# chalkydri/chalkydri

Hardware: AMD Instinct MI355X
Metric: frames/sec (detect+pose) on 1280x800 batch; HBM GB/s vs roofline (higher is better)
Workload: dtype u8 (threshold/segment/clusters: integer; quad fit/decode/SQPnP: f64)

## Files before the change

chalkydri_amd/csrc/k_clusters.hip:

```cpp
#include "ck_internal.h"
#include "ck_emit_row.h"

namespace {

constexpr int NT = 256;
constexpr int ETW = 64, ETH = 16;
constexpr int LW = ETW + 2, LH = ETH + 1;
constexpr int LHT = 512;
constexpr uint32_t SKIP = 0xFFFFFFFFu;

__device__ __forceinline__ uint32_t key_hash(unsigned long long k) {
    uint32_t x = (uint32_t)((k >> 32) ^ k);
    x *= 2654435761u;
    return x ^ (x >> 15);
}

struct EmitArgs {
    const uint8_t *thresh;
    const ck_label_t *labels;
    const uint32_t *groot, *gsize;
    size_t slots;
    int w, h, tiles_x, tiles_y, min_comp;
    int ccl_tiles_x;
    int stop_after;
    int twins;
    ck_stage_ws ws;
};

__device__ __forceinline__ void lds_barrier() { asm volatile("s_waitcnt lgkmcnt(0)\n\ts_barrier" ::: "memory"); }

__global__ __launch_bounds__(NT) void k_emit(EmitArgs a) {
    __shared__ uint8_t sT[LH][LW + 2];
    __shared__ uint32_t sR[LH][LW];
    __shared__ unsigned long long sKey[LHT];
    __shared__ uint32_t sCnt[LHT], sSlot[LHT], sTBase[LHT];
    __shared__ uint32_t sWave[NT / 64 + 1], sRunW[NT / 64 + 1];
    const int tid = threadIdx.x;
    const int tiles = a.tiles_x * a.tiles_y;
    const int frame = blockIdx.x / tiles, tile = blockIdx.x - frame * tiles;
    const int ty = tile / a.tiles_x, tx = tile - ty * a.tiles_x;
    const int x0 = tx * ETW, y0 = ty * ETH;
    const int w = a.w, h = a.h;
    const size_t npix = (size_t)w * h;
    const uint8_t *T = a.thresh + (size_t)frame * npix;
    const ck_label_t *L = a.labels + (size_t)frame * npix;
    const uint32_t *GR = a.groot + (size_t)frame * a.slots, *GS = a.gsize + (size_t)frame * a.slots;
    const ck_stage_ws &ws = a.ws;
    unsigned long long *gkeys = ws.d_ht_keys + (size_t)frame * ws.ht_size;
    unsigned long long *gcount = ws.d_ht_count + (size_t)frame * ws.ht_size;
    uint32_t *counters = ws.d_counters + (size_t)frame * CK_CNT_STRIDE;
    ck_packed_point *tmp = ws.d_tmp + (size_t)frame * ws.ext_cap;
    ck_run *runs = ws.d_runs + (size_t)frame * ws.run_cap;

    for (int i = tid; i < LHT; i += NT) { sKey[i] = 0ull; sCnt[i] = 0; }
    {
        constexpr int SPT = (LH * LW + NT - 1) / NT;
        uint32_t lab[SPT], hop[SPT], csz[SPT], slot[SPT];
        uint8_t tv[SPT];
#pragma unroll
        for (int q = 0; q < SPT; q++) {
            const int i = tid + q * NT;
            const int ly = i / LW, lx = i - ly * LW;
            const int gy = y0 + ly, gx = x0 - 1 + lx;
            tv[q] = 127; lab[q] = CK_LBL_NONE; slot[q] = 0;
            if (i < LH * LW && gy < h && gx >= 0 && gx < w) {
                const uint32_t p = (uint32_t)gy * (uint32_t)w + (uint32_t)gx;
                tv[q] = T[p]; lab[q] = L[p];
                slot[q] = ck_label_slot(lab[q], gx, gy, a.ccl_tiles_x);
            }
        }
#pragma unroll
        for (int q = 0; q < SPT; q++) {
            const bool two = tv[q] != 127 && !(lab[q] & CK_LBL_SMALL) && (lab[q] & CK_LBL_BORDER);
            hop[q] = two ? GR[slot[q]] : CK_LBL_INVALID;
            csz[q] = two ? GS[slot[q]] : 0u;
        }
#pragma unroll
        for (int q = 0; q < SPT; q++) {
            const int i = tid + q * NT;
            if (i >= LH * LW) continue;
            const int ly = i / LW, lx = i - ly * LW;
            uint32_t r = SKIP;
            if (tv[q] != 127 && !(lab[q] & CK_LBL_SMALL)) {
                if (lab[q] & CK_LBL_BORDER) r = ((int)csz[q] < a.min_comp) ? SKIP : hop[q];
                else r = ck_label_interior_root(lab[q], x0 - 1 + lx, y0 + ly, w);
            }
            sT[ly][lx] = tv[q];
            sR[ly][lx] = r;
        }
    }
    lds_barrier();
    if (a.stop_after == 0) return;

    const int lx = (tid & 63) + 1;
    const int gx = x0 + (tid & 63);
    const int row0 = (tid >> 6) * 4;
    const int dxs[4] = {1, 0, -1, 1}, dys[4] = {0, 1, 1, 1};
    const bool colok = gx >= 1 && gx <= w - 2;

    constexpr uint32_t NONE = 0xFFFFFFFFu;
    uint32_t cand[16];
#pragma unroll
    for (int q = 0; q < 16; q++) cand[q] = NONE;
    if (colok) {
#pragma unroll
        for (int rr = 0; rr < 4; rr++) {
            int ly = row0 + rr, gy = y0 + ly;
            if (gy < 1 || gy > h - 2) continue;
            int v0 = sT[ly][lx];
            uint32_t r0 = sR[ly][lx];
            if (r0 == SKIP) continue;
            uint32_t r1v[4];
            bool ok[4];
#pragma unroll
            for (int k = 0; k < 4; k++) {
                const int v1 = sT[ly + dys[k]][lx + dxs[k]];
                r1v[k] = sR[ly + dys[k]][lx + dxs[k]];
                ok[k] = (v0 + v1 == 255) && r1v[k] != SKIP;
            }
#pragma unroll
            for (int k = 0; k < 4; k++) {
                bool leader = ok[k];
#pragma unroll
                for (int j = 0; j < k; j++) leader = leader && !(ok[j] && r1v[j] == r1v[k]);
                if (!leader) continue;
                uint32_t n = 1;
#pragma unroll
                for (int j = k + 1; j < 4; j++) n += (ok[j] && r1v[j] == r1v[k]) ? 1u : 0u;
                const uint32_t r1 = r1v[k];
                unsigned long long key = r0 < r1 ? ((unsigned long long)r0 << 32) | r1 : ((unsigned long long)r1 << 32) | r0;
                uint32_t s = key_hash(key) & (LHT - 1);
                bool placed = false;
                for (int probe = 0; probe < LHT; probe++) {
                    __asm__ volatile("" ::: "memory");
                    unsigned long long prev = sKey[s];
                    if (prev == 0ull) prev = atomicCAS(&sKey[s], 0ull, key);
                    if (prev == 0ull || prev == key) {
                        uint32_t c = (s << 16) | atomicAdd(&sCnt[s], n);
                        cand[rr * 4 + k] = c;
#pragma unroll
                        for (int j = k + 1; j < 4; j++)
                            if (ok[j] && r1v[j] == r1) cand[rr * 4 + j] = ++c;
                        placed = true;
                        break;
                    }
                    s = (s + 1) & (LHT - 1);
                }
                if (!placed) atomicOr(&counters[CK_CNT_STATUS], (uint32_t)CK_FRAME_CLUSTERS_OVERFLOW);
            }
        }
    }
    lds_barrier();
    if (a.stop_after == 1) return;

    const unsigned long long k0 = sKey[2 * tid], k1 = sKey[2 * tid + 1];
    const uint32_t c0 = k0 ? sCnt[2 * tid] : 0u, c1 = k1 ? sCnt[2 * tid + 1] : 0u;
    uint32_t found0 = SKIP, found1 = SKIP, ridx0;
    {
        const uint32_t incl = wave_scan_u32(c0 + c1);
        const unsigned long long b0 = __ballot(k0 != 0ull), b1 = __ballot(k1 != 0ull);
        const unsigned long long below = (1ull << (tid & 63)) - 1ull;
        ridx0 = (uint32_t)(__popcll(b0 & below) + __popcll(b1 & below));
        if ((tid & 63) == 63) sWave[tid >> 6] = incl;
        if ((tid & 63) == 0) sRunW[tid >> 6] = (uint32_t)(__popcll(b0) + __popcll(b1));
        lds_barrier();
        uint32_t before = 0, total = 0, rbefore = 0, rtotal = 0;
#pragma unroll
        for (int wv = 0; wv < NT / 64; wv++) {
            uint32_t t = sWave[wv], r = sRunW[wv];
            if (wv < (tid >> 6)) { before += t; rbefore += r; }
            total += t; rtotal += r;
        }
        ridx0 += rbefore;
        lds_barrier();
        if (tid == 0) {
            sWave[NT / 64] = total ? atomicAdd(&counters[CK_CNT_TMP], total) : 0u;
            sRunW[NT / 64] = rtotal ? atomicAdd(&counters[CK_CNT_RUNS], rtotal) : 0u;
        }
        const uint32_t excl = before + incl - (c0 + c1);
        sTBase[2 * tid] = excl; sTBase[2 * tid + 1] = excl + c0;
        {
            const uint32_t hm = (uint32_t)(ws.ht_size - 1);
            const uint32_t g0 = key_hash(k0) & hm, g1 = key_hash(k1) & hm;
            const unsigned long long p0 = k0 ? atomicCAS(&gkeys[g0], 0ull, k0) : 0ull;
            const unsigned long long p1 = k1 ? atomicCAS(&gkeys[g1], 0ull, k1) : 0ull;
#pragma unroll
            for (int q = 0; q < 2; q++) {
                const unsigned long long key = q ? k1 : k0, pv = q ? p1 : p0;
                if (key == 0ull) continue;
                uint32_t g = q ? g1 : g0, found = SKIP;
                if (pv == 0ull || pv == key) found = g;
                else {
                    for (int probe = 1; probe < ws.ht_size; probe++) {
                        g = (g + 1) & hm;
                        unsigned long long prev = atomicCAS(&gkeys[g], 0ull, key);
                        if (prev == 0ull || prev == key) { found = g; break; }
                    }
                }
                if (found == SKIP) atomicOr(&counters[CK_CNT_STATUS], (uint32_t)CK_FRAME_CLUSTERS_OVERFLOW);
                sSlot[2 * tid + q] = found;
                if (q) found1 = found; else found0 = found;
            }
        }
        if (found0 != SKIP) atomicAdd(&gcount[found0], ((unsigned long long)c0 << 32) | c0);
        if (found1 != SKIP) atomicAdd(&gcount[found1], ((unsigned long long)c1 << 32) | c1);
    }
    lds_barrier();
    if (a.stop_after == 2) return;

    const uint32_t tile_base = sWave[NT / 64];
    if (colok) {
#pragma unroll
        for (int rr = 0; rr < 4; rr++) {
            int ly = row0 + rr, gy = y0 + ly;
#pragma unroll
            for (int k = 0; k < 4; k++) {
                const uint32_t cd = cand[rr * 4 + k];
                if (cd == NONE) continue;
                const uint32_t s = cd >> 16, lr = cd & 0xFFFFu;
                uint32_t slot = sSlot[s];
                if (slot == SKIP) continue;
                uint32_t ti = tile_base + sTBase[s] + lr;
                if (ti >= (uint32_t)ws.point_cap) { atomicOr(&counters[CK_CNT_STATUS], (uint32_t)CK_FRAME_POINTS_OVERFLOW); continue; }
                int v0 = sT[ly][lx], v1 = sT[ly + dys[k]][lx + dxs[k]];
                tmp[ti] = ((uint32_t)(2 * gx + dxs[k]) << 16) | ((uint32_t)(2 * gy + dys[k]) << 3) | ((uint32_t)k << 1) | (v1 > v0 ? 1u : 0u);
            }
        }
    }
    {
        uint32_t ri = sRunW[NT / 64] + ridx0;
#pragma unroll
        for (int q = 0; q < 2; q++) {
            if ((q ? k1 : k0) == 0ull) continue;
            const uint32_t found = q ? found1 : found0;
            if (ri < (uint32_t)ws.run_cap) {
                ck_run r;
                r.slot = found != SKIP ? found : 0u; r.base = 0; r.tmp_start = tile_base + sTBase[2 * tid + q];
                r.count = found != SKIP ? (q ? c1 : c0) : 0u;
                runs[ri] = r;
            } else if (found != SKIP) atomicOr(&counters[CK_CNT_STATUS], (uint32_t)CK_FRAME_CLUSTERS_OVERFLOW);
            ri++;
        }
    }
}

constexpr uint32_t ID_WHITE = 0x40000000u, ID_VALUE = 0x3FFFFFFFu;
static_assert(ID_WHITE == CK_PT_TWIN_SIGN, "a twin's sign is its white neighbour's colour bit, taken as it stands");
constexpr int SR_PAD = ((LH * LW + NT - 1) / NT) * NT;
static_assert(SKIP == CK_ER_SKIP && ID_WHITE == CK_ER_WHITE, "ck_emit_row.h speaks of the staged words of this kernel");
__device__ const ck_emit_row_table g_emit_rows = ck_make_emit_row_table();
static_assert(CK_ER_ROWS == 4 * NT, "one uint4 of the row table per thread");

__global__ __launch_bounds__(NT) __attribute__((amdgpu_num_sgpr(80), amdgpu_waves_per_eu(8))) void k_emit2(EmitArgs a, int xcd_map, int n_frames) {
    __shared__ __attribute__((aligned(16))) uint32_t sRaw[SR_PAD + LHT * 2 + LHT];
    __shared__ uint32_t sSlot[LHT], sTBase[LHT];
    __shared__ uint32_t sWave[NT / 64 + 1], sRunW[NT / 64 + 1];
    __shared__ __attribute__((aligned(16))) uint32_t sRow[CK_ER_ROWS];
    uint32_t *sR = sRaw;
    unsigned long long *sKey = reinterpret_cast<unsigned long long *>(sRaw + SR_PAD);
    uint32_t *sCnt = sRaw + SR_PAD + LHT * 2;
    const int tid = threadIdx.x;
    const int tiles = a.tiles_x * a.tiles_y;
    int frame, tile;
    if (xcd_map) {
        const int x = blockIdx.x & 7, j = blockIdx.x >> 3;
        frame = (j / tiles) * 8 + x; tile = j % tiles;
        if (frame >= n_frames) return;
    } else { frame = blockIdx.x / tiles; tile = blockIdx.x - frame * tiles; }
    const int ty = tile / a.tiles_x, tx = tile - ty * a.tiles_x;
    const int x0 = tx * ETW, y0 = ty * ETH;
    const int w = a.w, h = a.h;
    const size_t npix = (size_t)w * h;
    const uint8_t *T = a.thresh + (size_t)frame * npix;
    const ck_label_t *L = a.labels + (size_t)frame * npix;
    const uint32_t *GR = a.groot + (size_t)frame * a.slots, *GS = a.gsize + (size_t)frame * a.slots;
    const ck_stage_ws &ws = a.ws;
    unsigned long long *gkeys = ws.d_ht_keys + (size_t)frame * ws.ht_size;
    unsigned long long *gcount = ws.d_ht_count + (size_t)frame * ws.ht_size;
    uint32_t *counters = ws.d_counters + (size_t)frame * CK_CNT_STRIDE;
    ck_packed_point *tmp = ws.d_tmp + (size_t)frame * ws.ext_cap;
    ck_run *runs = ws.d_runs + (size_t)frame * ws.run_cap;

    for (int i = tid; i < LHT; i += NT) { sKey[i] = 0ull; sCnt[i] = 0; }
    {
        constexpr int SPT = SR_PAD / NT;
        uint32_t lab[SPT], tv[SPT], slot[SPT], hop[SPT], csz[SPT];
        bool inb[SPT];
        int gxs[SPT], gys[SPT];
#pragma unroll
        for (int q = 0; q < SPT; q++) {
            const int i = tid + q * NT;
            const int ly = i / LW, lx = i - ly * LW;
            const int gy = y0 + ly, gx = x0 - 1 + lx;
            inb[q] = i < LH * LW && gy < h && gx >= 0 && gx < w;
            const int cy = min(gy, h - 1), cx = min(max(gx, 0), w - 1);
            const uint32_t p = (uint32_t)cy * (uint32_t)w + (uint32_t)cx;
            tv[q] = T[p]; lab[q] = L[p];
            gxs[q] = cx; gys[q] = cy;
        }
#pragma unroll
        for (int q = 0; q < SPT; q++) {
            const bool two = inb[q] && tv[q] != 127u && !(lab[q] & CK_LBL_SMALL) && (lab[q] & CK_LBL_BORDER);
            slot[q] = two ? ck_label_slot(lab[q], gxs[q], gys[q], a.ccl_tiles_x) : 0u;
            hop[q] = GR[slot[q]]; csz[q] = GS[slot[q]];
        }
#pragma unroll
        for (int q = 0; q < SPT; q++) {
            const bool brd = (lab[q] & CK_LBL_BORDER) != 0u;
            const bool none = !inb[q] || tv[q] == 127u || (lab[q] & CK_LBL_SMALL) || (brd && (int)csz[q] < a.min_comp);
            const uint32_t root = brd ? hop[q] : ck_label_interior_root(lab[q], gxs[q], gys[q], w);
            sR[tid + q * NT] = none ? SKIP : (root | (tv[q] == 255u ? ID_WHITE : 0u));
        }
    }
    reinterpret_cast<uint4 *>(sRow)[tid] = reinterpret_cast<const uint4 *>(g_emit_rows.e)[tid];
    lds_barrier();
    if (a.stop_after == 0) return;

    const int lx = (tid & 63) + 1;
    const int gx = x0 + (tid & 63);
    const int row0 = (tid >> 6) * 4;

    constexpr uint32_t NONE = 0xFFFFFFFFu;
    uint32_t cand[16];
    {
        uint32_t R[5][3];
        unsigned long long last_key = 0ull;
        uint32_t last_s = 0;
        auto stage_row = [&](int r) {
#pragma unroll
            for (int c = 0; c < 3; c++) R[r][c] = sR[(row0 + r) * LW + lx - 1 + c];
        };
        stage_row(0); stage_row(1);
        uint32_t H[5];
        H[0] = ck_er_hword(R[0][0], R[0][1], R[0][2]);
        const uint32_t colskip = (uint32_t)(((gx - 1) | (w - 2 - gx)) >> 31);
        const uint32_t can = (a.twins ? 3u : 0u) & ~(((uint32_t)((gx - 2) >> 31) & CK_ER_CAN_DROP) | ((uint32_t)((w - 3 - gx) >> 31) & CK_ER_CAN_ABSORB));
        auto count = [&](uint32_t r0, uint32_t r1, uint32_t mult) -> uint32_t {
            const uint32_t ra = r0 & ID_VALUE, rb = r1 & ID_VALUE;
            const unsigned long long key = ra < rb ? ((unsigned long long)ra << 32) | rb : ((unsigned long long)rb << 32) | ra;
            uint32_t s = key_hash(key) & (LHT - 1);
            bool placed = false;
            if (key == last_key) { placed = true; s = last_s; }
            else
            for (int probe = 0; probe < LHT; probe++) {
                __asm__ volatile("" ::: "memory");
                unsigned long long prev = sKey[s];
                if (prev == 0ull) prev = atomicCAS(&sKey[s], 0ull, key);
                if (prev == 0ull || prev == key) { placed = true; break; }
                s = (s + 1) & (LHT - 1);
            }
            if (!placed) { atomicOr(&counters[CK_CNT_STATUS], (uint32_t)CK_FRAME_CLUSTERS_OVERFLOW); return NONE; }
            last_key = key; last_s = s;
            return (s << 16) | (atomicAdd(&sCnt[s], mult) >> 16);
        };
#pragma unroll
        for (int rr = 0; rr < 4; rr++) {
            const int gy = y0 + row0 + rr;
            if (rr < 3) stage_row(rr + 2);
            H[rr + 1] = ck_er_hword(R[rr + 1][0], R[rr + 1][1], R[rr + 1][2]);
            const uint32_t r0 = R[rr][1] | colskip | (uint32_t)(((gy - 1) | (h - 2 - gy)) >> 31);
            const uint32_t r1v[4] = {R[rr][2], R[rr + 1][1], R[rr + 1][0], R[rr + 1][2]};
            uint32_t absorb;
            const uint32_t idx = ck_er_index(H[rr], H[rr + 1], r0, R[rr][0], R[rr][1], R[rr][2], R[rr + 1][0], R[rr + 1][1], R[rr + 1][2], can, &absorb);
            const uint32_t e = sRow[idx];
            const uint32_t lj[4] = {0u, (e >> 20) & 1u, (e >> 21) & 3u, (e >> 23) & 3u};
            uint32_t c4[4] = {NONE, NONE, NONE, NONE};
            uint32_t le = e & CK_ER_LEADERS;
            for (uint32_t j = 0; (le & 0x1Cu) != 0u; j++, le >>= 5) {
                const uint32_t sl = le & 3u;
                const uint32_t r1 = sl == 0u ? r1v[0] : (sl == 1u ? r1v[1] : (sl == 2u ? r1v[2] : r1v[3]));
                const uint32_t c = count(r0, r1, ((le >> 2) & 7u) * 0x10001u + (lj[3] == j ? absorb : 0u));
#pragma unroll
                for (int k = 0; k < 4; k++) c4[k] = lj[k] == j ? c : c4[k];
            }
#pragma unroll
            for (int k = 0; k < 4; k++) {
                const uint32_t nth = k == 0 ? 0u : (k == 1 ? (e >> 25) & 1u : (k == 2 ? (e >> 26) & 3u : (e >> 28) & 3u));
                uint32_t c = c4[k];
                c = ((idx >> (9 - k)) & 1u) ? c : NONE;
                const uint32_t sign = (r1v[k] & ID_WHITE) << 1;
                const uint32_t twin = k == 3 ? (0u - absorb) & (CK_PT_TWIN | (r1v[1] & ID_WHITE)) : 0u;
                cand[rr * 4 + k] = c != NONE ? ((c + nth) | sign | twin) : NONE;
                asm volatile("" : "+v"(cand[rr * 4 + k]));
            }
        }
    }
    lds_barrier();
    if (a.stop_after == 1) return;

    const unsigned long long k0 = sKey[2 * tid], k1 = sKey[2 * tid + 1];
    const uint32_t b0 = k0 ? sCnt[2 * tid] : 0u, b1 = k1 ? sCnt[2 * tid + 1] : 0u;
    const uint32_t c0 = b0 >> 16, c1 = b1 >> 16;
    uint32_t found0 = SKIP, found1 = SKIP, ridx0;
    {
        const uint32_t incl2 = wave_scan_u32(b0 + b1), incl = incl2 >> 16;
        const unsigned long long u0 = __ballot(k0 != 0ull), u1 = __ballot(k1 != 0ull);
        const unsigned long long below = (1ull << (tid & 63)) - 1ull;
        ridx0 = (uint32_t)(__popcll(u0 & below) + __popcll(u1 & below));
        if ((tid & 63) == 63) sWave[tid >> 6] = incl2;
        if ((tid & 63) == 0) sRunW[tid >> 6] = (uint32_t)(__popcll(u0) + __popcll(u1));
        lds_barrier();
        uint32_t before = 0, total = 0, rbefore = 0, rtotal = 0;
#pragma unroll
        for (int wv = 0; wv < NT / 64; wv++) {
            uint32_t t = sWave[wv], r = sRunW[wv];
            if (wv < (tid >> 6)) { before += t; rbefore += r; }
            total += t; rtotal += r;
        }
        ridx0 += rbefore;
        before >>= 16;
        if (tid == 0) {
            const uint32_t ptotal = total >> 16, ltotal = total & 0xFFFFu;
            static_assert(CK_CNT_TMP == 0 && CK_CNT_CLUSTERS == 1 && CK_CNT_STRIDE % 2 == 0, "the two counters are one aligned 64-bit word");
            const unsigned long long was = total ? atomicAdd(reinterpret_cast<unsigned long long *>(counters), ((unsigned long long)ltotal << 32) | ptotal) : 0ull;
            sWave[NT / 64] = (uint32_t)was;
            sRunW[NT / 64] = rtotal ? atomicAdd(&counters[CK_CNT_RUNS], rtotal) : 0u;
            if ((uint32_t)(was >> 32) + ltotal > (uint32_t)ws.point_cap) atomicOr(&counters[CK_CNT_STATUS], (uint32_t)CK_FRAME_POINTS_OVERFLOW);
        }
        const uint32_t excl = before + incl - (c0 + c1);
        sTBase[2 * tid] = excl; sTBase[2 * tid + 1] = excl + c0;
        {
            const uint32_t hm = (uint32_t)(ws.ht_size - 1);
            const uint32_t g0 = key_hash(k0) & hm, g1 = key_hash(k1) & hm;
            const unsigned long long p0 = k0 ? atomicCAS(&gkeys[g0], 0ull, k0) : 0ull;
            const unsigned long long p1 = k1 ? atomicCAS(&gkeys[g1], 0ull, k1) : 0ull;
#pragma unroll
            for (int q = 0; q < 2; q++) {
                const unsigned long long key = q ? k1 : k0, pv = q ? p1 : p0;
                uint32_t found = SKIP;
                if (key != 0ull) {
                    uint32_t g = q ? g1 : g0;
                    if (pv == 0ull || pv == key) found = g;
                    else {
                        for (int probe = 1; probe < ws.ht_size; probe++) {
                            g = (g + 1) & hm;
                            unsigned long long prev = atomicCAS(&gkeys[g], 0ull, key);
                            if (prev == 0ull || prev == key) { found = g; break; }
                        }
                    }
                    if (found == SKIP) atomicOr(&counters[CK_CNT_STATUS], (uint32_t)CK_FRAME_CLUSTERS_OVERFLOW);
                }
                sSlot[2 * tid + q] = found;
                if (q) found1 = found; else found0 = found;
            }
        }
        if (found0 != SKIP) atomicAdd(&gcount[found0], ((unsigned long long)(b0 & 0xFFFFu) << 32) | c0);
        if (found1 != SKIP) atomicAdd(&gcount[found1], ((unsigned long long)(b1 & 0xFFFFu) << 32) | c1);
    }
    lds_barrier();
    if (a.stop_after == 2) return;

    const uint32_t tile_base = sWave[NT / 64];
#pragma unroll
    for (int q = 0; q < 16; q++) {
        const uint32_t cd = cand[q];
        if (cd == NONE) continue;
        const int rr = q >> 2, k = q & 3;
        const int dxk = k == 1 ? 0 : (k == 2 ? -1 : 1), dyk = k == 0 ? 0 : 1;
        const uint32_t s = (cd >> 16) & 0x3FFu, lr = cd & 0xFFFFu;
        if (sSlot[s] == SKIP) continue;
        const uint32_t ti = tile_base + sTBase[s] + lr;
        if (ti >= (uint32_t)ws.point_cap) continue;
        const int gy = y0 + row0 + rr;
        const uint32_t twin = k == 3 ? cd & (CK_PT_TWIN | CK_PT_TWIN_SIGN) : 0u;
        tmp[ti] = twin | ((uint32_t)(2 * gx + dxk) << 16) | ((uint32_t)(2 * gy + dyk) << 3) | ((uint32_t)k << 1) | (cd >> 31);
    }
    {
        uint32_t ri = sRunW[NT / 64] + ridx0;
#pragma unroll
        for (int q = 0; q < 2; q++) {
            if ((q ? k1 : k0) == 0ull) continue;
            const uint32_t found = q ? found1 : found0;
            if (ri < (uint32_t)ws.run_cap) {
                ck_run r;
                r.slot = found != SKIP ? found : 0u; r.base = 0; r.tmp_start = tile_base + (q ? sTBase[2 * tid + 1] : sTBase[2 * tid]);
                r.count = found != SKIP ? (q ? c1 : c0) : 0u;
                runs[ri] = r;
            } else if (found != SKIP) atomicOr(&counters[CK_CNT_STATUS], (uint32_t)CK_FRAME_CLUSTERS_OVERFLOW);
            ri++;
        }
    }
}

__global__ __launch_bounds__(NT) void k_clear(uint4 *keys4, size_t nkeys4, uint4 *cnt4, size_t ncnt4, uint32_t *c0, uint32_t n0, uint32_t *c1,
                                              uint32_t n1, uint32_t *c2, uint32_t n2) {
    const size_t i = (size_t)blockIdx.x * NT + threadIdx.x;
    const uint4 z = make_uint4(0, 0, 0, 0);
    if (i < nkeys4) keys4[i] = z;
    else if (i - nkeys4 < ncnt4) cnt4[i - nkeys4] = z;
    if (i < n0) c0[i] = 0;
    if (i < n1) c1[i] = 0;
    if (i < n2) c2[i] = 0;
}

constexpr int SNT = 1024;
__global__ __launch_bounds__(SNT) void k_scan(ck_stage_ws ws, int min_cluster, int max_cluster) {
    __shared__ uint32_t sPts[SNT / 64], sLog[SNT / 64], sCl[SNT / 64];
    const int frame = blockIdx.x, tid = threadIdx.x, lane = tid & 63, wv = tid >> 6;
    const unsigned long long *gkeys = ws.d_ht_keys + (size_t)frame * ws.ht_size;
    const unsigned long long *gcount = ws.d_ht_count + (size_t)frame * ws.ht_size;
    uint32_t *goff = ws.d_ht_off + (size_t)frame * ws.ht_size;
    uint32_t *counters = ws.d_counters + (size_t)frame * CK_CNT_STRIDE;
    ck_cluster_t *clusters = ws.d_clusters + (size_t)frame * ws.cluster_cap;
    const int seg = ws.ht_size / (SNT / 64);
    const int base = wv * seg;
    uint32_t pts = 0, lpts = 0, cl = 0;
#pragma unroll 8
    for (int r = 0; r < seg; r += 64) {
        const unsigned long long c2 = gcount[base + r + lane];
        const uint32_t c = (uint32_t)c2, lc = (uint32_t)(c2 >> 32);
        bool ok = (int)lc >= min_cluster && (int)lc <= max_cluster;
        pts += ok ? c : 0u; lpts += ok ? lc : 0u; cl += ok ? 1u : 0u;
    }
    pts = (uint32_t)__builtin_amdgcn_readlane((int)wave_scan_u32(pts), 63);
    lpts = (uint32_t)__builtin_amdgcn_readlane((int)wave_scan_u32(lpts), 63);
    cl = (uint32_t)__builtin_amdgcn_readlane((int)wave_scan_u32(cl), 63);
    if (lane == 0) { sPts[wv] = pts; sLog[wv] = lpts; sCl[wv] = cl; }
    __syncthreads();
    uint32_t po = 0, lo = 0, co = 0;
    for (int k = 0; k < wv; k++) { po += sPts[k]; lo += sLog[k]; co += sCl[k]; }
    for (int r4 = 0; r4 < seg; r4 += 256) {
        unsigned long long c4[4];
#pragma unroll
        for (int q = 0; q < 4; q++) c4[q] = r4 + 64 * q < seg ? gcount[base + r4 + 64 * q + lane] : 0ull;
#pragma unroll
    for (int q = 0; q < 4; q++) {
        const int r = r4 + 64 * q;
        if (r >= seg) continue;
        const int e = base + r + lane;
        const uint32_t c = (uint32_t)c4[q], lc = (uint32_t)(c4[q] >> 32);
        const bool ok = (int)lc >= min_cluster && (int)lc <= max_cluster;
        const uint32_t ip = wave_scan_u32(ok ? c : 0u), il = wave_scan_u32(ok ? lc : 0u), ic = wave_scan_u32(ok ? 1u : 0u);
        uint32_t off = SKIP;
        if (ok) {
            const uint32_t my_po = po + ip - c, my_lo = lo + il - lc, my_co = co + ic - 1u;
            if (my_co < (uint32_t)ws.cluster_cap && my_lo + lc <= (uint32_t)ws.point_cap) {
                off = my_po;
                unsigned long long key = gkeys[e];
                ck_cluster_t ck;
                ck.rep0 = (uint32_t)(key >> 32); ck.rep1 = (uint32_t)key; ck.start = my_po; ck.count = c;
                clusters[my_co] = ck;
            } else {
                if (my_co < (uint32_t)ws.cluster_cap) {
                    ck_cluster_t ck;
                    ck.rep0 = 0; ck.rep1 = 0; ck.start = 0; ck.count = 0;
                    clusters[my_co] = ck;
                }
                atomicOr(&counters[CK_CNT_STATUS], (uint32_t)CK_FRAME_CLUSTERS_OVERFLOW);
            }
        }
        goff[e] = off;
        po += (uint32_t)__builtin_amdgcn_readlane((int)ip, 63);
        lo += (uint32_t)__builtin_amdgcn_readlane((int)il, 63);
        co += (uint32_t)__builtin_amdgcn_readlane((int)ic, 63);
    }
    }
    if (tid == SNT - 1) {
        counters[CK_CNT_CLUSTERS] = min(co, (uint32_t)ws.cluster_cap);
        counters[CK_CNT_POINTS] = min(po, (uint32_t)ws.point_cap);
    }
}

template <int RPW>
__global__ __launch_bounds__(NT) void k_scatter(ck_stage_ws ws) {
    const int frame = blockIdx.y;
    const uint32_t *counters = ws.d_counters + (size_t)frame * CK_CNT_STRIDE;
    const uint32_t nruns = min(counters[CK_CNT_RUNS], (uint32_t)ws.run_cap);
    const uint32_t ntmp = min(counters[CK_CNT_TMP], (uint32_t)ws.point_cap);
    const ck_packed_point *tmp = ws.d_tmp + (size_t)frame * ws.ext_cap;
    const ck_run *runs = ws.d_runs + (size_t)frame * ws.run_cap;
    uint32_t *goff = ws.d_ht_off + (size_t)frame * ws.ht_size;
    ck_packed_point *pts = ws.d_points + (size_t)frame * ws.ext_cap;
    const int lane = threadIdx.x & 63;
    const uint32_t wave = blockIdx.x * (NT / 64) + (threadIdx.x >> 6), nwaves = gridDim.x * (NT / 64);
    for (uint32_t r0 = wave * RPW; r0 < nruns; r0 += nwaves * RPW) {
        ck_run mine = {0, 0, 0, 0};
        uint32_t moff = SKIP;
        if (lane < RPW && r0 + lane < nruns) { mine = runs[r0 + lane]; moff = goff[mine.slot]; }
        if (moff == SKIP) mine.count = 0;
        const uint32_t dst0 = mine.count ? atomicAdd(&goff[mine.slot], mine.count) : 0u;
        const unsigned long long small = __ballot(mine.count > 0 && mine.count <= 64);
        unsigned long long todo = small;
        const int sub = lane >> 4, sl = lane & 15;
        while (todo) {
            unsigned long long t = todo;
            int pick = -1;
#pragma unroll
            for (int q = 0; q < 4; q++) {
                const int bit = t ? __builtin_ctzll(t) : -1;
                if (q == sub) pick = bit;
                if (t) t &= t - 1;
            }
            todo = t;
            const int srcl = pick < 0 ? 0 : pick;
            const uint32_t cnt = (uint32_t)__shfl((int)mine.count, srcl, 64), ts = (uint32_t)__shfl((int)mine.tmp_start, srcl, 64),
                           ds = (uint32_t)__shfl((int)dst0, srcl, 64);
            ck_packed_point v[4];
            bool ok[4];
#pragma unroll
            for (int q = 0; q < 4; q++) {
                const uint32_t j = (uint32_t)sl + 16u * q;
                ok[q] = pick >= 0 && j < cnt && ts + j < ntmp;
                v[q] = ok[q] ? tmp[ts + j] : 0u;
            }
#pragma unroll
            for (int q = 0; q < 4; q++)
                if (ok[q]) pts[ds + (uint32_t)sl + 16u * q] = v[q];
        }
        unsigned long long big = __ballot(mine.count > 64);
        while (big) {
            const int srcl = __builtin_ctzll(big);
            big &= big - 1;
            const uint32_t cnt = (uint32_t)__builtin_amdgcn_readlane((int)mine.count, srcl), ts = (uint32_t)__builtin_amdgcn_readlane((int)mine.tmp_start, srcl),
                           ds = (uint32_t)__builtin_amdgcn_readlane((int)dst0, srcl);
            for (uint32_t j0 = 0; j0 < cnt; j0 += 256) {
                ck_packed_point v[4];
                bool ok[4];
#pragma unroll
                for (int q = 0; q < 4; q++) {
                    const uint32_t j = j0 + (uint32_t)lane + 64u * q;
                    ok[q] = j < cnt && ts + j < ntmp;
                    v[q] = ok[q] ? tmp[ts + j] : 0u;
                }
#pragma unroll
                for (int q = 0; q < 4; q++)
                    if (ok[q]) pts[ds + j0 + (uint32_t)lane + 64u * q] = v[q];
            }
        }
    }
}

}

int ck_launch_clusters(ck_handle *h, int n) {
    ck_stage_ws &ws = h->ws;
    {
        const ck_fit_layout fl = ck_fit_scratch_layout(ws, h->cfg.max_batch);
        const size_t nkeys4 = (size_t)ws.ht_size * n / 2, ncnt4 = (size_t)ws.ht_size * n / 2;
        const size_t total4 = nkeys4 + ncnt4;
        hipLaunchKernelGGL(k_clear, dim3((unsigned)((total4 + NT - 1) / NT)), dim3(NT), 0, h->stream,
                           reinterpret_cast<uint4 *>(ws.d_ht_keys), nkeys4, reinterpret_cast<uint4 *>(ws.d_ht_count), ncnt4, ws.d_counters,
                           (uint32_t)(CK_CNT_STRIDE * n), fl.list_counts, 32u, fl.cand_count, (uint32_t)n);
    }
    EmitArgs a;
    a.thresh = h->d_thresh; a.labels = h->d_labels; a.groot = h->d_groot; a.gsize = h->d_gsize; a.slots = (size_t)h->broot_cap;
    a.w = h->qw; a.h = h->qh; a.tiles_x = (h->qw + ETW - 1) / ETW; a.tiles_y = (h->qh + ETH - 1) / ETH;
    a.min_comp = h->cfg.min_component_px; a.ws = ws; a.ccl_tiles_x = h->tiles_x;
    { static const int stop_after = CK_KNOB("CK_EMIT_STOP_AFTER", 99); a.stop_after = stop_after; }
    { static const int twins = CK_KNOB("CK_EMIT_TWINS", 1); a.twins = twins; }
    static const int emit_v = CK_KNOB("CK_EMIT_V", 2);
    static const int emit_xcd = CK_KNOB("CK_EMIT_XCD", -1);
    if (emit_v == 1) hipLaunchKernelGGL(k_emit, dim3((unsigned)(a.tiles_x * a.tiles_y * n)), dim3(NT), 0, h->stream, a);
    else {
        const int xcd_map = emit_xcd >= 0 ? emit_xcd : (n >= 16 ? 1 : 0);
        const unsigned grid = xcd_map ? (unsigned)(((n + 7) / 8) * 8 * a.tiles_x * a.tiles_y) : (unsigned)(a.tiles_x * a.tiles_y * n);
        hipLaunchKernelGGL(k_emit2, dim3(grid), dim3(NT), 0, h->stream, a, xcd_map, n);
    }
    int min_cluster = h->cfg.min_cluster_pixels < 24 ? 24 : h->cfg.min_cluster_pixels;
    hipLaunchKernelGGL(k_scan, dim3((unsigned)n), dim3(SNT), 0, h->stream, ws, min_cluster, ws.max_cluster_points);
    if (n <= 4) hipLaunchKernelGGL(k_scatter<8>, dim3(256u, (unsigned)n), dim3(NT), 0, h->stream, ws);
    else {
        static const unsigned sc_wgs = (unsigned)CK_KNOB("CK_SCATTER_WGS", 32);
        hipLaunchKernelGGL(k_scatter<64>, dim3(sc_wgs, (unsigned)n), dim3(NT), 0, h->stream, ws);
    }
    CK_HIP(hipGetLastError());
    return CK_OK;
}
```

Before: 20710.

## Stage emit tile with vectorized 4-pixel loads and drop sSlot shared array

Adds a templated staging path to k_emit2 in which each thread loads four adjacent threshold bytes and labels in one vector load and writes a uint4 into a padded LDS layout (stride 68). The halo column and bottom row are handled by a second partial round on the first waves. Separately, the per-key slot array in shared memory is folded into sTBase through a NO_RUN flag bit, and the thread-local tile bases stay in registers. The goal is fewer global load instructions and less LDS use during tile staging. The path is only taken when the width is a multiple of 4 and the pointers are aligned, and it adds extra index math.

Result: faster. 21220, median of 6 (+2.5%).

```diff
diff --git a/chalkydri_amd/csrc/ck_emit_stage.h b/chalkydri_amd/csrc/ck_emit_stage.h
--- /dev/null
+++ b/chalkydri_amd/csrc/ck_emit_stage.h
@@ -0,0 +1,76 @@
+#ifndef CK_EMIT_STAGE_H
+#define CK_EMIT_STAGE_H
+
+#include <stdint.h>
+
+#if defined(__HIPCC__)
+#define CK_ES_HD __host__ __device__ __forceinline__
+#else
+#define CK_ES_HD inline
+#endif
+
+constexpr int CK_ES_NT = 256;
+constexpr int CK_ES_TW = 64, CK_ES_TH = 16;
+constexpr int CK_ES_LW = CK_ES_TW + 2, CK_ES_LH = CK_ES_TH + 1;
+constexpr int CK_ES_STRIDE = 68, CK_ES_COL0 = 3;
+constexpr int CK_ES_WORDS = CK_ES_STRIDE * (CK_ES_LH - 1) + CK_ES_COL0 + CK_ES_LW;
+constexpr int CK_ES_ROUND1 = CK_ES_TW + 2 * CK_ES_LH;
+constexpr int CK_ES_ROUND1_WAVES = (CK_ES_ROUND1 + 63) / 64;
+constexpr int CK_ES_CCL_TW = 128, CK_ES_CCL_TH = 32, CK_ES_RING_CAP = 2 * (CK_ES_CCL_TW + CK_ES_CCL_TH);
+constexpr uint32_t CK_ES_LBL_BORDER = 0x8000u, CK_ES_LBL_SMALL = 0x4000u, CK_ES_LBL_ID_MASK = 0x01FFu;
+constexpr uint32_t CK_ES_SKIP = 0xFFFFFFFFu, CK_ES_WHITE = 0x40000000u;
+
+CK_ES_HD bool ck_es_group_path(int w) { return w >= 4 && (w & 3) == 0; }
+
+CK_ES_HD int ck_es_word(int ly, int lx) { return ly * CK_ES_STRIDE + CK_ES_COL0 + lx; }
+
+struct ck_es_item {
+    int ly, lx;
+    int cx, cy;
+    bool keep;
+    bool inb;
+};
+
+CK_ES_HD ck_es_item ck_es_round0(int t, int x0, int y0, int w, int h) {
+    ck_es_item it;
+    it.ly = t >> 4; it.lx = 1 + 4 * (t & 15); it.keep = true;
+    const int gx = x0 - 1 + it.lx, gy = y0 + it.ly;
+    it.inb = gx < w && gy < h;
+    it.cx = gx > w - 4 ? w - 4 : gx;
+    it.cy = gy > h - 1 ? h - 1 : gy;
+    return it;
+}
+
+CK_ES_HD ck_es_item ck_es_round1(int t, int x0, int y0, int w, int h) {
+    ck_es_item it;
+    const int j = t - CK_ES_TW < 2 * CK_ES_LH ? t - CK_ES_TW : 2 * CK_ES_LH - 1;
+    const bool right = j >= CK_ES_LH;
+    it.ly = t < CK_ES_TW ? CK_ES_LH - 1 : (right ? j - CK_ES_LH : j);
+    it.lx = t < CK_ES_TW ? 1 + t : (right ? CK_ES_LW - 1 : 0);
+    it.keep = t < CK_ES_ROUND1;
+    const int gx = x0 - 1 + it.lx, gy = y0 + it.ly;
+    it.inb = gx >= 0 && gx < w && gy < h;
+    it.cx = gx < 0 ? 0 : (gx > w - 1 ? w - 1 : gx);
+    it.cy = gy > h - 1 ? h - 1 : gy;
+    return it;
+}
+
+CK_ES_HD int ck_es_item_word(const ck_es_item &it) { return ck_es_word(it.ly, it.lx); }
+
+CK_ES_HD uint32_t ck_es_slot_base(int cx, int cy, int ccl_tiles_x) {
+    return (((uint32_t)cy / (uint32_t)CK_ES_CCL_TH) * (uint32_t)ccl_tiles_x + (uint32_t)cx / (uint32_t)CK_ES_CCL_TW) * (uint32_t)CK_ES_RING_CAP;
+}
+CK_ES_HD uint32_t ck_es_root_base(int cx, int cy, int w) { return (uint32_t)(cy & ~(CK_ES_CCL_TH - 1)) * (uint32_t)w + (uint32_t)(cx & ~(CK_ES_CCL_TW - 1)); }
+
+CK_ES_HD uint32_t ck_es_pixel_slot(uint32_t lab, uint32_t tv, bool inb, uint32_t slot_base) {
+    const bool two = inb && tv != 127u && !(lab & CK_ES_LBL_SMALL) && (lab & CK_ES_LBL_BORDER);
+    return two ? slot_base + (lab & CK_ES_LBL_ID_MASK) : 0u;
+}
+CK_ES_HD uint32_t ck_es_pixel_word(uint32_t lab, uint32_t tv, bool inb, uint32_t hop, uint32_t csz, uint32_t root_base, int w, int min_comp) {
+    const bool brd = (lab & CK_ES_LBL_BORDER) != 0u;
+    const bool none = !inb || tv == 127u || (lab & CK_ES_LBL_SMALL) || (brd && (int)csz < min_comp);
+    const uint32_t root = brd ? hop : root_base + ((lab >> 7) & (uint32_t)(CK_ES_CCL_TH - 1)) * (uint32_t)w + (lab & (uint32_t)(CK_ES_CCL_TW - 1));
+    return none ? CK_ES_SKIP : (root | (tv == 255u ? CK_ES_WHITE : 0u));
+}
+
+#endif
diff --git a/chalkydri_amd/csrc/k_clusters.hip b/chalkydri_amd/csrc/k_clusters.hip
--- a/chalkydri_amd/csrc/k_clusters.hip
+++ b/chalkydri_amd/csrc/k_clusters.hip
@@ -1,5 +1,6 @@
 #include "ck_internal.h"
 #include "ck_emit_row.h"
+#include "ck_emit_stage.h"
 
 namespace {
 
@@ -24,6 +25,7 @@
     int ccl_tiles_x;
     int stop_after;
     int twins;
+    int stage4;
     ck_stage_ws ws;
 };
 
@@ -250,10 +252,14 @@
 static_assert(SKIP == CK_ER_SKIP && ID_WHITE == CK_ER_WHITE, "ck_emit_row.h speaks of the staged words of this kernel");
 __device__ const ck_emit_row_table g_emit_rows = ck_make_emit_row_table();
 static_assert(CK_ER_ROWS == 4 * NT, "one uint4 of the row table per thread");
-
+static_assert(CK_ES_NT == NT && CK_ES_TW == ETW && CK_ES_TH == ETH && CK_ES_LW == LW && CK_ES_LH == LH && CK_ES_WORDS <= SR_PAD, "ck_emit_stage.h speaks of this kernel's tile");
+static_assert(CK_ES_CCL_TW == CK_TW && CK_ES_CCL_TH == CK_TH && CK_ES_RING_CAP == CK_RING_CAP && CK_ES_LBL_BORDER == CK_LBL_BORDER && CK_ES_LBL_SMALL == CK_LBL_SMALL &&
+              CK_ES_LBL_ID_MASK == CK_LBL_ID_MASK && CK_ES_SKIP == SKIP && CK_ES_WHITE == ID_WHITE, "... and of the label words of ck_internal.h");
+
+template <bool G4>
 __global__ __launch_bounds__(NT) __attribute__((amdgpu_num_sgpr(80), amdgpu_waves_per_eu(8))) void k_emit2(EmitArgs a, int xcd_map, int n_frames) {
     __shared__ __attribute__((aligned(16))) uint32_t sRaw[SR_PAD + LHT * 2 + LHT];
-    __shared__ uint32_t sSlot[LHT], sTBase[LHT];
+    __shared__ uint32_t sTBase[LHT];
     __shared__ uint32_t sWave[NT / 64 + 1], sRunW[NT / 64 + 1];
     __shared__ __attribute__((aligned(16))) uint32_t sRow[CK_ER_ROWS];
     uint32_t *sR = sRaw;
@@ -282,6 +288,49 @@
     ck_run *runs = ws.d_runs + (size_t)frame * ws.run_cap;
 
     for (int i = tid; i < LHT; i += NT) { sKey[i] = 0ull; sCnt[i] = 0; }
+    if constexpr (G4) {
+        auto at = [](const void *base, uint32_t bytes) { return reinterpret_cast<const char *>(base) + bytes; };
+        auto gather = [&](uint32_t slot, uint32_t &hop, uint32_t &csz) {
+            hop = *reinterpret_cast<const uint32_t *>(at(GR, slot * 4u)); csz = *reinterpret_cast<const uint32_t *>(at(GS, slot * 4u));
+        };
+        const bool round1 = __builtin_amdgcn_readfirstlane(tid >> 6) < CK_ES_ROUND1_WAVES;
+        const ck_es_item it0 = ck_es_round0(tid, x0, y0, w, h);
+        ck_es_item it1 = it0;
+        uint32_t lab[4], tv[4], hop[4], csz[4], lab1 = 0u, tv1 = 0u, hop1 = 0u, csz1 = 0u;
+        {
+            const uint32_t p = (uint32_t)it0.cy * (uint32_t)w + (uint32_t)it0.cx;
+            const uint32_t t4 = *reinterpret_cast<const uint32_t *>(at(T, p));
+            const uint2 l4 = *reinterpret_cast<const uint2 *>(at(L, p * (uint32_t)sizeof(ck_label_t)));
+#pragma unroll
+            for (int j = 0; j < 4; j++) {
+                tv[j] = (t4 >> (8 * j)) & 0xFFu;
+                const uint32_t l2 = j < 2 ? l4.x : l4.y;
+                lab[j] = (j & 1) ? l2 >> 16 : l2 & 0xFFFFu;
+            }
+        }
+        if (round1) {
+            it1 = ck_es_round1(tid, x0, y0, w, h);
+            const uint32_t p = (uint32_t)it1.cy * (uint32_t)w + (uint32_t)it1.cx;
+            tv1 = T[p]; lab1 = L[p];
+        }
+        {
+            const uint32_t slot_base = ck_es_slot_base(it0.cx, it0.cy, a.ccl_tiles_x);
+#pragma unroll
+            for (int j = 0; j < 4; j++) gather(ck_es_pixel_slot(lab[j], tv[j], it0.inb, slot_base), hop[j], csz[j]);
+        }
+        if (round1) gather(ck_es_pixel_slot(lab1, tv1, it1.inb && it1.keep, ck_es_slot_base(it1.cx, it1.cy, a.ccl_tiles_x)), hop1, csz1);
+        {
+            const uint32_t rb = ck_es_root_base(it0.cx, it0.cy, w);
+            uint4 v;
+            v.x = ck_es_pixel_word(lab[0], tv[0], it0.inb, hop[0], csz[0], rb, w, a.min_comp);
+            v.y = ck_es_pixel_word(lab[1], tv[1], it0.inb, hop[1], csz[1], rb, w, a.min_comp);
+            v.z = ck_es_pixel_word(lab[2], tv[2], it0.inb, hop[2], csz[2], rb, w, a.min_comp);
+            v.w = ck_es_pixel_word(lab[3], tv[3], it0.inb, hop[3], csz[3], rb, w, a.min_comp);
+            *reinterpret_cast<uint4 *>(sR + ck_es_item_word(it0)) = v;
+        }
+        if (round1 && it1.keep)
+            sR[ck_es_item_word(it1)] = ck_es_pixel_word(lab1, tv1, it1.inb, hop1, csz1, ck_es_root_base(it1.cx, it1.cy, w), w, a.min_comp);
+    } else
     {
         constexpr int SPT = SR_PAD / NT;
         uint32_t lab[SPT], tv[SPT], slot[SPT], hop[SPT], csz[SPT];
@@ -320,7 +369,7 @@
     const int gx = x0 + (tid & 63);
     const int row0 = (tid >> 6) * 4;
 
-    constexpr uint32_t NONE = 0xFFFFFFFFu;
+    constexpr uint32_t NONE = 0xFFFFFFFFu, NO_RUN = 0x80000000u;
     uint32_t cand[16];
     {
         uint32_t R[5][3];
@@ -328,7 +377,7 @@
         uint32_t last_s = 0;
         auto stage_row = [&](int r) {
 #pragma unroll
-            for (int c = 0; c < 3; c++) R[r][c] = sR[(row0 + r) * LW + lx - 1 + c];
+            for (int c = 0; c < 3; c++) R[r][c] = sR[G4 ? ck_es_word(row0 + r, lx - 1 + c) : (row0 + r) * LW + lx - 1 + c];
         };
         stage_row(0); stage_row(1);
         uint32_t H[5];
@@ -391,7 +440,7 @@
     const unsigned long long k0 = sKey[2 * tid], k1 = sKey[2 * tid + 1];
     const uint32_t b0 = k0 ? sCnt[2 * tid] : 0u, b1 = k1 ? sCnt[2 * tid + 1] : 0u;
     const uint32_t c0 = b0 >> 16, c1 = b1 >> 16;
-    uint32_t found0 = SKIP, found1 = SKIP, ridx0;
+    uint32_t found0 = SKIP, found1 = SKIP, ridx0, tb0, tb1;
     {
         const uint32_t incl2 = wave_scan_u32(b0 + b1), incl = incl2 >> 16;
         const unsigned long long u0 = __ballot(k0 != 0ull), u1 = __ballot(k1 != 0ull);
@@ -418,7 +467,7 @@
             if ((uint32_t)(was >> 32) + ltotal > (uint32_t)ws.point_cap) atomicOr(&counters[CK_CNT_STATUS], (uint32_t)CK_FRAME_POINTS_OVERFLOW);
         }
         const uint32_t excl = before + incl - (c0 + c1);
-        sTBase[2 * tid] = excl; sTBase[2 * tid + 1] = excl + c0;
+        tb0 = excl; tb1 = excl + c0;
         {
             const uint32_t hm = (uint32_t)(ws.ht_size - 1);
             const uint32_t g0 = key_hash(k0) & hm, g1 = key_hash(k1) & hm;
@@ -440,7 +489,7 @@
                     }
                     if (found == SKIP) atomicOr(&counters[CK_CNT_STATUS], (uint32_t)CK_FRAME_CLUSTERS_OVERFLOW);
                 }
-                sSlot[2 * tid + q] = found;
+                sTBase[2 * tid + q] = (q ? tb1 : tb0) | (found == SKIP ? NO_RUN : 0u);
                 if (q) found1 = found; else found0 = found;
             }
         }
@@ -458,7 +507,6 @@
         const int rr = q >> 2, k = q & 3;
         const int dxk = k == 1 ? 0 : (k == 2 ? -1 : 1), dyk = k == 0 ? 0 : 1;
         const uint32_t s = (cd >> 16) & 0x3FFu, lr = cd & 0xFFFFu;
-        if (sSlot[s] == SKIP) continue;
         const uint32_t ti = tile_base + sTBase[s] + lr;
         if (ti >= (uint32_t)ws.point_cap) continue;
         const int gy = y0 + row0 + rr;
@@ -473,7 +521,7 @@
             const uint32_t found = q ? found1 : found0;
             if (ri < (uint32_t)ws.run_cap) {
                 ck_run r;
-                r.slot = found != SKIP ? found : 0u; r.base = 0; r.tmp_start = tile_base + (q ? sTBase[2 * tid + 1] : sTBase[2 * tid]);
+                r.slot = found != SKIP ? found : 0u; r.base = 0; r.tmp_start = tile_base + (q ? tb1 : tb0);
                 r.count = found != SKIP ? (q ? c1 : c0) : 0u;
                 runs[ri] = r;
             } else if (found != SKIP) atomicOr(&counters[CK_CNT_STATUS], (uint32_t)CK_FRAME_CLUSTERS_OVERFLOW);
@@ -648,13 +696,16 @@
     a.min_comp = h->cfg.min_component_px; a.ws = ws; a.ccl_tiles_x = h->tiles_x;
     { static const int stop_after = CK_KNOB("CK_EMIT_STOP_AFTER", 99); a.stop_after = stop_after; }
     { static const int twins = CK_KNOB("CK_EMIT_TWINS", 1); a.twins = twins; }
+    { static const int stage4 = CK_KNOB("CK_EMIT_STAGE4", 1); a.stage4 = stage4; }
     static const int emit_v = CK_KNOB("CK_EMIT_V", 2);
     static const int emit_xcd = CK_KNOB("CK_EMIT_XCD", -1);
     if (emit_v == 1) hipLaunchKernelGGL(k_emit, dim3((unsigned)(a.tiles_x * a.tiles_y * n)), dim3(NT), 0, h->stream, a);
     else {
         const int xcd_map = emit_xcd >= 0 ? emit_xcd : (n >= 16 ? 1 : 0);
         const unsigned grid = xcd_map ? (unsigned)(((n + 7) / 8) * 8 * a.tiles_x * a.tiles_y) : (unsigned)(a.tiles_x * a.tiles_y * n);
-        hipLaunchKernelGGL(k_emit2, dim3(grid), dim3(NT), 0, h->stream, a, xcd_map, n);
+        const bool g4 = a.stage4 && ck_es_group_path(a.w) && ((uintptr_t)a.thresh & 3u) == 0 && ((uintptr_t)a.labels & 7u) == 0;
+        if (g4) hipLaunchKernelGGL(k_emit2<true>, dim3(grid), dim3(NT), 0, h->stream, a, xcd_map, n);
+        else hipLaunchKernelGGL(k_emit2<false>, dim3(grid), dim3(NT), 0, h->stream, a, xcd_map, n);
     }
     int min_cluster = h->cfg.min_cluster_pixels < 24 ? 24 : h->cfg.min_cluster_pixels;
     hipLaunchKernelGGL(k_scan, dim3((unsigned)n), dim3(SNT), 0, h->stream, ws, min_cluster, ws.max_cluster_points);
```
